# zju3dv/LoG

Measured on NVIDIA H100. Metric: gaussians_per_s_fwd_bwd, higher is better.
Workload: dtype f32

## Files before the change

### include/log_b200_raster.h

```cpp
#ifndef LOG_B200_RASTER_H
#define LOG_B200_RASTER_H

#include <stdint.h>

#ifdef __cplusplus
extern "C" {
#endif

#define LGR_ABI_VERSION 27
#define LGR_TILE 16

#define LGR_FILTER_ADD 0
#define LGR_FILTER_MAX 1
#define LGR_FILTER_NONE 2

#define LGR_E_BADARG (-1)
#define LGR_E_CAPACITY (-2)
#define LGR_E_UNSUPPORTED (-3)

typedef struct lgr_view {
  int32_t image_height, image_width;
  float tanfovx, tanfovy;
  float scale_modifier;
  int32_t sh_degree;
  int32_t sh_coeffs;
  int32_t filter_mode;
  int32_t want_aux;
  int32_t tile_row_begin, tile_row_end;
  int32_t num_owners;
  int32_t raw_params;
  int32_t* band_ids_d;
  int32_t* band_blk_d;
  int32_t* band_count_d;
  int32_t* band_rows_d;
  float* band_dsplat_d;
  int32_t* tile_rank_d;
  const int64_t* gather_index_d;
  const int32_t* pid_map_d;
  int32_t* contrib_id_d;
  uint32_t* contrib_entry_d;
  int32_t* contrib_count_d;
  const int32_t* last_contrib_d;
  const int32_t* region_count_d;
  int64_t region_cap;
  int32_t num_regions;
  int32_t num_channels;
  int32_t log_depth;
  float* splat_ext_d;
  const float* cov3D_precomp_d;
  float* dcov3D_d;
  const float* viewmatrix_d;
  const float* projmatrix_d;
  const float* campos_d;
  const float* bg_d;
} lgr_view;

#define LGR_SPLAT_FLOATS 12
#define LGR_GRAD_FLOATS 12
#define LGR_TILE_SCRATCH_INTS 33
#define LGR_CONTRIB_MAX_LIST (1 << 24)
#define LGR_META_INTS 8

int lgr_abi_version(void);

int lgr_compute_radius(int64_t n, const float* means3D_d, const float* scales_d, const float* rotations_d,
                       const float* projmatrix_d, const float* viewmatrix_d, float focal_x, float focal_y,
                       float tan_fovx, float tan_fovy, float* radii_d, void* stream);

int lgr_mark_visible(int64_t n, const float* means3D_d, const float* viewmatrix_d, uint8_t* visible_d, void* stream);

int lgr_forward_project(const lgr_view* view, int64_t n, const float* means3D_d, const float* opacities_d,
                        const float* scales_d, const float* rotations_d, const float* colors_precomp_d,
                        const float* shs_d, float* splat_d, int32_t* radii_d, uint8_t* clamped_d,
                        int32_t* tile_start_d, int32_t* tile_cursor_d, int32_t* meta_d, void* stream);

int lgr_forward_render(const lgr_view* view, int64_t n, int64_t num_instances, int32_t max_tile_len,
                       int32_t num_long_tiles, const float* splat_d, const int32_t* radii_d, const int32_t* tile_start_d,
                       int32_t* tile_cursor_d, uint32_t* inst_key_d, uint32_t* inst_val_d, uint32_t* inst_tmp_d,
                       int32_t* sorted_ids_d, float* image_d, float* final_T_d, int32_t* n_contrib_d,
                       int32_t* point_id_pixel_d, float* point_weight_pixel_d, float* point_weight_d,
                       int32_t* point_count_d, void* stream);
int32_t lgr_sort_smem_capacity(void);

int lgr_forward_render_device_sized(const lgr_view* view, int64_t n, int64_t instance_capacity, int32_t* meta_d,
                                    const float* splat_d, const int32_t* radii_d, int32_t* tile_start_d,
                                    int32_t* tile_cursor_d, uint32_t* inst_key_d, uint32_t* inst_val_d,
                                    uint32_t* inst_tmp_d, int32_t* sorted_ids_d, float* image_d, float* final_T_d, int32_t* n_contrib_d,
// ... 231 lines not shown
```

### log_b200/_capi.py

```python
import ctypes
import os

from .build import LIB_PATH

_i32, _i64, _f32, _vp = ctypes.c_int32, ctypes.c_int64, ctypes.c_float, ctypes.c_void_p

LGR_FILTER_ADD, LGR_FILTER_MAX, LGR_FILTER_NONE = 0, 1, 2
LGR_SPLAT_FLOATS = 12
LGR_GRAD_FLOATS = 12
LGR_META_INTS = 8
LGR_TILE_SCRATCH_INTS = 33
LGR_ABI_VERSION = 27
LGR_CONTRIB_MAX_LIST = 1 << 24
LGR_STAGE_HEADER_FLOATS = 64
LGR_ROW_FLOATS = 20

EXPORTS = ('lgr_abi_version', 'lgr_sort_smem_capacity', 'lgr_compute_radius', 'lgr_forward_project',
           'lgr_forward_render', 'lgr_forward_render_device_sized', 'lgr_backward', 'lgr_grad_scatter_add', 'lgr_grad_scatter_add_staged', 'lgr_point_compact', 'lgr_sparse_adam', 'lgr_profile_enable', 'lgr_profile_collect',
           'lgr_profile_kernel_name', 'lgr_shard_send', 'lgr_shard_recv_bin', 'lgr_blend_backward', 'lgr_shard_return_rows',
           'lgr_shard_gather', 'lgr_shard_recv_bin_aux', 'lgr_shard_return_packed', 'lgr_shard_gather_packed', 'lgr_tree_traverse', 'lgr_mark_visible',
           'lgr_ssim_forward', 'lgr_ssim_backward', 'lgr_depth_loss_forward', 'lgr_depth_loss_backward', 'lgr_depth_vis',
           'lgr_counter_update', 'lgr_log_step', 'lgr_prepare_cull', 'lgr_prepare_select', 'lgr_photometric_forward',
           'lgr_photometric_backward', 'lgr_corrector_step', 'lgr_densify_plan', 'lgr_densify_map', 'lgr_densify_children',
           'lgr_densify_gather', 'lgr_step_order')
LGR_SHARD_MAX_RANKS = 32
LGR_PROFILE_KERNELS = 12


class LgrView(ctypes.Structure):
    _fields_ = [('image_height', _i32), ('image_width', _i32), ('tanfovx', _f32), ('tanfovy', _f32),
                ('scale_modifier', _f32), ('sh_degree', _i32), ('sh_coeffs', _i32), ('filter_mode', _i32),
                ('want_aux', _i32), ('tile_row_begin', _i32), ('tile_row_end', _i32),
                ('num_owners', _i32), ('raw_params', _i32), ('band_ids_d', _vp), ('band_blk_d', _vp), ('band_count_d', _vp), ('band_rows_d', _vp), ('band_dsplat_d', _vp), ('tile_rank_d', _vp), ('gather_index_d', _vp), ('pid_map_d', _vp), ('contrib_id_d', _vp), ('contrib_entry_d', _vp), ('contrib_count_d', _vp), ('last_contrib_d', _vp),
                ('region_count_d', _vp), ('region_cap', _i64), ('num_regions', _i32), ('num_channels', _i32), ('log_depth', _i32), ('splat_ext_d', _vp), ('cov3D_precomp_d', _vp), ('dcov3D_d', _vp),
                ('viewmatrix_d', _vp), ('projmatrix_d', _vp), ('campos_d', _vp), ('bg_d', _vp)]


class LgrShardLayout(ctypes.Structure):
    _fields_ = [('num_ranks', _i32), ('my_rank', _i32), ('cap', _i64), ('off_count', _i64), ('off_splat', _i64),
                ('off_radii', _i64), ('off_gid', _i64), ('off_dsplat', _i64), ('off_weight', _i64), ('off_pcount', _i64)]


class LgrTree(ctypes.Structure):
    _fields_ = [('num_points', _i64), ('num_nodes', _i64), ('max_child', _i32), ('max_level', _i32),
                ('node_index_d', _vp), ('tree_d', _vp)]


def tree_scratch_ints(num_points, slots):
    return 8 + 2 * num_points + slots + 2 * ((slots + 255) // 256) + 2 + (slots + 3) // 4


class LgrPrepare(ctypes.Structure):
    _fields_ = [('num_points', _i64), ('num_roots', _i64), ('xyz_d', _vp), ('full_proj_d', _vp), ('bound_lo', _f32),
                ('bound_hi', _f32), ('root_index_d', _vp), ('node_index_d', _vp), ('depth_d', _vp), ('opt_all_levels', _i32),
                ('current_depth', _i32), ('flag_d', _vp), ('in_range_d', _vp), ('roots_d', _vp), ('index_all_d', _vp),
                ('leaf_d', _vp), ('node_d', _vp), ('result_d', _vp), ('scratch_d', _vp)]


LGR_PREPARE_RESULTS = 8
(LGR_PREPARE_IN_RANGE, LGR_PREPARE_ROOTS, LGR_PREPARE_WALK, LGR_PREPARE_LEAVES, LGR_PREPARE_NODES, LGR_PREPARE_STATUS,
 LGR_PREPARE_INSTANCES, LGR_PREPARE_OVERFLOW) = range(8)
LGR_PREPARE_ROOT_ORDER = 1


def prepare_scratch_ints(num_points, slots):
    return 2 * num_points + 2 * ((num_points + 255) // 256) + 2 + (num_points + 3) // 4 + tree_scratch_ints(num_points, slots)


# ... 206 lines not shown
```

### log_b200/csrc/lgr_capi.cu

```cuda
#include "lgr_common.cuh"
#include "lgr_prof.cuh"
#include <math.h>

namespace lgr {
int launch_mark_visible(int64_t, const float*, const float*, uint8_t*, cudaStream_t);
int launch_compute_radius(int64_t, const float*, const float*, const float*, const float*, const float*, float, float,
                          float, float, float*, cudaStream_t);
int launch_project_fwd(const View&, Colour, bool, int64_t, const float*, const float*, const float*, const float*,
                       const float*, const float*, float*, int32_t*, uint8_t*, int32_t*, int32_t*, cudaStream_t);
int launch_project_bwd(const View&, Colour, bool, bool, int64_t, const float*, const float*, const float*, const float*,
                       const float*, const int32_t*, const uint8_t*, const float*, float*, float*, float*, float*, float*,
                       float*, float*, float*, void* const*, int, cudaStream_t);
int launch_grad_scatter_add(int64_t, const float*, int64_t, int64_t, float*, cudaStream_t);
int launch_grad_scatter_add_staged(const float*, int, int64_t, int64_t, int64_t, float*, cudaStream_t);
int launch_band_scan(const View&, cudaStream_t);
int launch_tile_scan(int, int32_t*, int32_t*, int32_t*, bool, cudaStream_t);
int launch_bin_and_sort(const View&, int64_t, int64_t, int, int, const float*, const int32_t*, int32_t*, int32_t*,
                        uint32_t*, uint32_t*, uint32_t*, int32_t*, int32_t*, cudaStream_t);
int sort_smem_capacity();
int launch_blend_fwd(const View&, const int32_t*, const int32_t*, const float*, float*, float*, int32_t*, int32_t*,
                     float*, float*, int32_t*, cudaStream_t);
int launch_sparse_adam(int64_t, int, const int64_t*, const float*, float*, float*, float*, float*, float, float, float, float,
                       float, float, float, cudaStream_t);
int launch_counter_update(const lgr_counter&, int64_t, int64_t, const int64_t*, const int64_t*, const int32_t*, const float*,
                          const float*, const int64_t*, int64_t, const void*, const void*, int, int, uint8_t*, cudaStream_t);
int launch_log_step(const lgr_step&, int64_t, int64_t, const int64_t*, const int64_t*, const uint8_t*, cudaStream_t);
int launch_step_order(int64_t, int64_t, int64_t, const int64_t*, const int64_t*, const uint8_t*, int32_t*, int64_t*, cudaStream_t);
int launch_point_compact(int64_t, const int32_t*, int32_t*, int32_t*, int32_t*, int32_t*, cudaStream_t);
int launch_blend_bwd(const View&, const int32_t*, const int32_t*, const float*, const float*, const float*, float*,
                     cudaStream_t);
int launch_shard_send(const View&, const ShardLayout&, int64_t, int64_t, const float*, const int32_t*, int32_t*, void* const*,
                      cudaStream_t);
int launch_shard_recv_count(const View&, const ShardLayout&, float*, float*, int32_t*, int32_t*, float*, int32_t*, cudaStream_t);
int launch_shard_return_packed(const ShardLayout&, const float*, const float*, const float*, const int32_t*, void* const*, cudaStream_t);
int launch_shard_return(const ShardLayout&, const float*, int64_t, const void*, int, int64_t, void* const*, cudaStream_t);
int launch_shard_gather(const View&, const ShardLayout&, int64_t, const float*, const int32_t*, const int32_t*, const float*,
                        float*, float*, int32_t*, int, cudaStream_t);
int launch_tree_traverse(const TreeArgs&, int64_t, int64_t, const int64_t*, int64_t, const int64_t*, int, int32_t*, int64_t*, int64_t*,
                         cudaStream_t);
int launch_prepare_cull(const lgr_prepare&, cudaStream_t);
int launch_prepare_select(const lgr_prepare&, const TreeArgs&, int64_t, int, const float*, const int32_t*, cudaStream_t);
int launch_ssim_fwd(int, int, int, int, const float*, const int64_t*, const float*, const int64_t*, double*, float*, float*,
// ... 190 lines not shown
}

int lgr_backward(const lgr_view* view, int64_t n, int64_t num_instances, const float* means3D_d,
                 const float* opacities_d, const float* scales_d, const float* rotations_d,
                 const float* colors_precomp_d, const float* shs_d, const float* splat_d, const int32_t* radii_d,
                 const uint8_t* clamped_d, const int32_t* tile_start_d, const int32_t* sorted_ids_d,
                 const float* image_d, const float* dL_dimage_d, float* dsplat_d,
                 float* dmeans3D_d, float* dmeans2D_d, float* dopacities_d, float* dscales_d, float* drotations_d,
                 float* dcolors_d, float* dshs_d, float* grad_rows_d, void* const* peer_stage_d, int32_t my_rank,
                 int64_t num_rows, void* stream) {
  if (!view_ok(view) || n < 0 || !tile_start_d || !image_d || !dL_dimage_d) return LGR_E_BADARG;
  if (const int rc6 = six_channels_check(view)) return rc6;
  const bool rows_mode = grad_rows_d || peer_stage_d;
  if (view->num_channels == 6 && rows_mode) return LGR_E_UNSUPPORTED;
  Colour c;
  if (const int rc = colour_source(view, n, colors_precomp_d, shs_d, &c)) return rc;
  if (n == 0) return 0;
  if (c == Colour::LOG_SH && (!dshs_d || !view->campos_d || view->num_owners > 0)) return LGR_E_BADARG;
  const bool cov3d = view->cov3D_precomp_d != nullptr;
  if (!means3D_d || (!cov3d && (!scales_d || !rotations_d)) || !splat_d || !radii_d || !dsplat_d) return LGR_E_BADARG;
  if (cov3d && (!view->dcov3D_d || view->raw_params || view->num_owners > 0 || grad_rows_d || peer_stage_d)) return LGR_E_BADARG;
  if (view->raw_params && (!opacities_d || c == Colour::SH)) return LGR_E_BADARG;
  if (rows_mode) {
    if (view->num_owners <= 0 || c == Colour::SH) return LGR_E_BADARG;
    if (peer_stage_d && (my_rank < 0 || my_rank >= view->num_owners)) return LGR_E_BADARG;
    if (num_rows < 0 || num_rows > n) return LGR_E_BADARG;
  } else {
    if (view->num_owners > 0) return LGR_E_BADARG;
    if (!dmeans3D_d || !dmeans2D_d || !dopacities_d || (!cov3d && (!dscales_d || !drotations_d))) return LGR_E_BADARG;
    if (c == Colour::SH ? (!dshs_d || !clamped_d || !view->campos_d) : !dcolors_d) return LGR_E_BADARG;
  }
  if (num_instances > 0 && !sorted_ids_d) return LGR_E_BADARG;
  cudaStream_t st = (cudaStream_t)stream;
  const View v = make_view(view, n);
  int rc = 0;
  if (num_instances > 0) rc = launch_blend_bwd(v, tile_start_d, sorted_ids_d, splat_d, image_d, dL_dimage_d, dsplat_d, st);
  if (rc) return rc;
  return launch_project_bwd(v, c, cov3d, rows_mode, rows_mode ? num_rows : n, means3D_d, opacities_d, scales_d, rotations_d, shs_d, radii_d, clamped_d, dsplat_d,
                            dmeans3D_d, dmeans2D_d, dopacities_d, dscales_d, drotations_d, dcolors_d, dshs_d, grad_rows_d, peer_stage_d, my_rank, st);
}

int lgr_sparse_adam(int64_t rows, int32_t row_floats, const int64_t* index_d, const float* grad_d, float* param_d,
                    float* exp_avg_d, float* exp_avg_sq_d, float* max_exp_avg_sq_d, int64_t step, double lr, double beta1,
                    double beta2, double eps, void* stream) {
  if (rows < 0 || row_floats <= 0 || step < 1) return LGR_E_BADARG;
  if (rows > 0 && (!index_d || !grad_d || !param_d || !exp_avg_d || !exp_avg_sq_d)) return LGR_E_BADARG;
  Residence where;
  where.on_device(param_d); where.on_device(index_d); where.on_device(grad_d);
  where.state(exp_avg_d); where.state(exp_avg_sq_d); where.state(max_exp_avg_sq_d);
  if (!where.ok) return LGR_E_BADARG;
  const double bc1 = 1.0 - pow(beta1, (double)step), bc2 = 1.0 - pow(beta2, (double)step);
  const double step_size = lr / bc1;
  return launch_sparse_adam(rows, row_floats, index_d, grad_d, param_d, exp_avg_d, exp_avg_sq_d, max_exp_avg_sq_d,
                            (float)beta1, (float)beta2, (float)(1.0 - beta1), (float)(1.0 - beta2), (float)sqrt(bc2),
                            (float)(-step_size), (float)eps, (cudaStream_t)stream);
}

int lgr_counter_update(const lgr_counter* counter, int64_t num_leaf, int64_t num_node, const int64_t* index_leaf_d,
                       const int64_t* index_node_d, const int32_t* radii_d, const float* point_weight_d, const float* grad_d,
                       const int64_t* grad_strides, int64_t num_points, const void* point_id_d, const void* point_count_d,
                       int32_t id_bytes, int32_t count_bytes, uint8_t* flag_vis_d, void* stream) {
  if (!counter || num_leaf < 0 || num_node < 0 || num_points < 0 || !grad_strides) return LGR_E_BADARG;
  if ((id_bytes != 4 && id_bytes != 8) || (count_bytes != 4 && count_bytes != 8)) return LGR_E_BADARG;
  if ((num_leaf > 0 && !index_leaf_d) || (num_node > 0 && !index_node_d)) return LGR_E_BADARG;
  const lgr_counter& c = *counter;
  if (!c.create_steps_d || !c.visible_count_d || !c.weights_max_d || !c.weights_sum_d || !c.radii_max_d || !c.area_sum_d ||
      !c.grad_sum_d || !c.radii_max_max_d)
    return LGR_E_BADARG;
// ... 416 lines not shown
```

### log_b200/csrc/lgr_common.cuh

```cuda
#pragma once
#include <cuda_runtime.h>
#include <stdint.h>

#include "../../include/log_b200_raster.h"

namespace lgr {

constexpr int TILE = LGR_TILE;
constexpr int TILE_PIX = TILE * TILE;
constexpr float NEAR_Z = 0.2f;
constexpr float ALPHA_MAX = 0.99f;
constexpr float ALPHA_MIN = 1.0f / 255.0f;
constexpr float T_STOP = 1e-4f;
constexpr float FILTER_VAR = 0.3f;
constexpr float CLAMP_FOV = 1.3f;
constexpr int CSTRIDE = 32;
constexpr float LOG2E = 1.4426950408889634f;
constexpr float LN2 = 0.6931471805599453f;
constexpr int COMPACT_CHUNK = 256;

enum class Colour { RGB, SH, LOG_SH, RGB6 };

struct View {
  int H, W, gx, gy;
  int row0, row1;
  float tanfovx, tanfovy, fx, fy, scale_mod;
  int sh_degree, sh_K, filter_mode, want_aux;
  int raw_params;
  int num_owners, owner_chunk;
  int32_t* band_ids;
  int32_t* band_blk;
  int32_t* band_count;
  int32_t* band_rows;
  float* band_dsplat;
  const int64_t* gather;
  const int32_t* pid_map;
  int32_t* contrib_id;
  uint32_t* contrib_entry;
  int32_t* contrib_count;
  const int32_t* last_contrib;
  const int32_t* region_count;
  int64_t region_cap;
  int regions;
  const float* cov3d;
  float* dcov3d;
  int band_blocks;
  const float* view;
  const float* proj;
  const float* campos;
  const float* bg;
  int num_channels;
  int log_depth;
  float* splat_ext;
};

inline View make_view(const lgr_view* v, int64_t n = 0) {
  View o;
  o.num_owners = v->num_owners; o.band_ids = v->band_ids_d; o.band_blk = v->band_blk_d; o.band_count = v->band_count_d; o.band_rows = v->band_rows_d; o.band_dsplat = v->band_dsplat_d; o.gather = v->gather_index_d; o.pid_map = v->pid_map_d; o.contrib_id = v->contrib_id_d; o.contrib_entry = v->contrib_entry_d; o.contrib_count = v->contrib_count_d; o.last_contrib = v->last_contrib_d;
  o.region_count = v->region_count_d; o.region_cap = v->region_cap; o.regions = v->region_count_d ? v->num_regions : 0;
  o.cov3d = v->cov3D_precomp_d; o.dcov3d = v->dcov3D_d;
  o.owner_chunk = o.num_owners > 0 ? (int)LGR_OWNER_CHUNK(n, (int64_t)o.num_owners) : 256;
  if (o.owner_chunk < 256) o.owner_chunk = 256;
  o.band_blocks = (int)((n + 255) / 256);
  o.H = v->image_height; o.W = v->image_width;
  o.gx = (o.W + TILE - 1) / TILE; o.gy = (o.H + TILE - 1) / TILE;
  o.row0 = v->tile_row_begin; o.row1 = v->tile_row_end;
  if (o.row0 == 0 && o.row1 == 0) o.row1 = o.gy;
  o.tanfovx = v->tanfovx; o.tanfovy = v->tanfovy;
  o.fx = o.W / (2.0f * v->tanfovx); o.fy = o.H / (2.0f * v->tanfovy);
  o.scale_mod = v->scale_modifier;
  o.sh_degree = v->sh_degree; o.sh_K = v->sh_coeffs; o.filter_mode = v->filter_mode; o.want_aux = v->want_aux;
  o.raw_params = v->raw_params;
  o.view = v->viewmatrix_d; o.proj = v->projmatrix_d; o.campos = v->campos_d; o.bg = v->bg_d;
  o.num_channels = v->num_channels == 6 ? 6 : 3; o.splat_ext = v->splat_ext_d; o.log_depth = v->log_depth ? 1 : 0;
  return o;
}

struct ShardLayout {
  int R, me;
  int64_t cap;
  int64_t off_count, off_splat, off_radii, off_gid, off_dsplat, off_weight, off_pcount;
};

struct TreeArgs {
  const int32_t* node_index;
  const int32_t* tree;
  int C;
  const float* xyz;
  const float* scaling_raw;
  const float* rotation_raw;
  const float* view;
  const float* proj;
  float fx, fy, tanfovx, tanfovy, min_px;
};


__device__ __forceinline__ float4 ldg4(const float* p) { return __ldg(reinterpret_cast<const float4*>(p)); }

struct Cov2D {
  float a, b, c;
  float a_raw, c_raw;
  float t[3];
  float T[6];
  bool inx, iny;
};

__device__ __forceinline__ void quat_to_R(const float4 q, float R[9]) {
// ... 179 lines not shown
```

### log_b200/csrc/lgr_project.cu

```cuda
#include "lgr_common.cuh"
#include "lgr_prof.cuh"

namespace lgr {

constexpr int PROJ_THREADS = 256;

__device__ __forceinline__ void load3(const float* __restrict__ p, int64_t i, float o[3]) {
  o[0] = __ldg(p + 3 * i); o[1] = __ldg(p + 3 * i + 1); o[2] = __ldg(p + 3 * i + 2);
}

__device__ __forceinline__ void load_cov3d(const float* cov, int64_t i, float Sg[9]) {
  const float* c6 = cov + 6 * i;
  const float cxx = __ldg(c6), cxy = __ldg(c6 + 1), cxz = __ldg(c6 + 2), cyy = __ldg(c6 + 3), cyz = __ldg(c6 + 4), czz = __ldg(c6 + 5);
  Sg[0] = cxx; Sg[1] = cxy; Sg[2] = cxz; Sg[3] = cxy; Sg[4] = cyy; Sg[5] = cyz; Sg[6] = cxz; Sg[7] = cyz; Sg[8] = czz;
}

__device__ __forceinline__ void sh_dir_basis(const float p[3], const float* cam, int deg, float B[16]) {
  const float d[3] = {p[0] - cam[0], p[1] - cam[1], p[2] - cam[2]};
  const float inv = 1.0f / sqrtf(d[0] * d[0] + d[1] * d[1] + d[2] * d[2]);
  sh_basis(deg, d[0] * inv, d[1] * inv, d[2] * inv, B);
}

__device__ __forceinline__ void sh_accumulate(const float* sh, const float B[16], int first, int nb, float rgb[3]) {
  for (int k = first; k < nb; k++) {
// ... 239 lines not shown
template <Colour C, bool COV3D, bool DEPTH, bool ROWS>
__global__ void __launch_bounds__(PROJ_THREADS)
project_bwd_kernel(View v, int64_t n, const float* __restrict__ means, const float* __restrict__ opac,
                   const float* __restrict__ scales, const float* __restrict__ rots, const float* __restrict__ shs, const int32_t* __restrict__ radii,
                   const uint8_t* __restrict__ clamped, const float* __restrict__ dsplat, float* __restrict__ dmeans,
                   float* __restrict__ dmeans2D, float* __restrict__ dopac, float* __restrict__ dscales,
                   float* __restrict__ drots, float* __restrict__ dcolors, float* __restrict__ dshs,
                   float* __restrict__ grad_rows, void* const* __restrict__ peer_stage, int my_rank) {
  static_assert(!(C == Colour::RGB6 && DEPTH), "the depth pass generates channels 3..5: colours are (N,3)");
  static_assert(!(C == Colour::LOG_SH && COV3D), "LoG's raw parameters come with scales and rotations");
  static_assert(!ROWS || (C == Colour::RGB && !COV3D && !DEPTH), "band mode rows carry three precomputed colours only");
  constexpr bool USE_SH = C == Colour::SH, LOG_SH = C == Colour::LOG_SH, SIX = C == Colour::RGB6;
  __shared__ float sV[16], sP[16], sCam[3];
  if (threadIdx.x < 16) { sV[threadIdx.x] = v.view[threadIdx.x]; sP[threadIdx.x] = v.proj[threadIdx.x]; }
  if ((USE_SH || LOG_SH) && threadIdx.x < 3) sCam[threadIdx.x] = v.campos[threadIdx.x];
  __syncthreads();
  int64_t blk = blockIdx.x;
  if (ROWS && peer_stage) {
    int64_t first = 0;
    for (int o = 0; o <= my_rank && o < v.num_owners - 1; o++) first += v.band_count[o];
    if (my_rank == v.num_owners - 1) first = 0;
    blk = (blk + first / PROJ_THREADS) % gridDim.x;
  }
  int64_t i = blk * PROJ_THREADS + threadIdx.x;
  const bool active = i < n;
  if (!ROWS && !active) return;
  int64_t row = 0;
  if (ROWS && active) {
    row = i;
    i = v.band_rows[row];
  }
  float dm[3] = {0.f, 0.f, 0.f}, dm2[2] = {0.f, 0.f}, dop = 0.f, dsc[3] = {0.f, 0.f, 0.f}, dq[4] = {0.f, 0.f, 0.f, 0.f};
  float drgb[3] = {0.f, 0.f, 0.f}, dext[3] = {0.f, 0.f, 0.f};
  const bool live = active && radii[i] > 0;
  const int64_t src = (v.gather && live) ? v.gather[i] : i;
  const int K = v.sh_K;
  if (live) {
    const float4 g0 = ldg4(dsplat + i * LGR_GRAD_FLOATS);
    const float4 g1 = ldg4(dsplat + i * LGR_GRAD_FLOATS + 4);
    const float4 g2 = ldg4(dsplat + i * LGR_GRAD_FLOATS + 8);
    float p[3], s0[3], s[3], R[9], Sg[9];
    load3(means, src, p);
    float4 q = make_float4(1.f, 0.f, 0.f, 0.f);
    float q_inv = 1.0f;
    if (COV3D) {
      load_cov3d(v.cov3d, src, Sg);
    } else {
      load3(scales, src, s0);
      q = ldg4(rots + 4 * src);
      if (v.raw_params) {
#pragma unroll
        for (int k = 0; k < 3; k++) s0[k] = expf(s0[k]);
        q = act_normalize(q, q_inv);
      }
#pragma unroll
      for (int k = 0; k < 3; k++) s[k] = s0[k] * v.scale_mod;
      quat_to_R(q, R);
      cov3d(s, R, Sg);
    }
    Cov2D cv;
    cov2d(sV, p, Sg, v.fx, v.fy, v.tanfovx, v.tanfovy, v.filter_mode, cv);
    dop = g1.y;
    drgb[0] = g1.z; drgb[1] = g1.w; drgb[2] = g2.x;
    if (SIX) { dext[0] = g2.y; dext[1] = g2.z; dext[2] = g2.w; }
    const float a = cv.a, b = cv.b, c = cv.c;
    const float det = a * c - b * b, idet2 = 1.0f / (det * det);
    float da = idet2 * (-c * c * g0.z + b * c * g0.w + (det - a * c) * g1.x);
// ... 167 lines not shown
      }
      float4* sr = s_rows + threadIdx.x * 5;
      sr[0] = make_float4(dm[0], dm[1], dm[2], dm2[0]);
      sr[1] = make_float4(dm2[1], 0.f, dop, dsc[0]);
      sr[2] = make_float4(dsc[1], dsc[2], dq[0], dq[1]);
      sr[3] = make_float4(dq[2], dq[3], drgb[0], drgb[1]);
      sr[4] = make_float4(drgb[2], __int_as_float((int)i), (float)radii[i], 0.f);
      s_dst[threadIdx.x] = dst;
    }
    __syncthreads();
    const int64_t left = n - blk * PROJ_THREADS;
    const int cnt = left < PROJ_THREADS ? (int)left : PROJ_THREADS;
    for (int idx = threadIdx.x; idx < cnt * 5; idx += PROJ_THREADS) {
      const int r = idx / 5;
      s_dst[r][idx - 5 * r] = s_rows[idx];
    }
    return;
  }
  dmeans[3 * i] = dm[0]; dmeans[3 * i + 1] = dm[1]; dmeans[3 * i + 2] = dm[2];
  dmeans2D[3 * i] = dm2[0]; dmeans2D[3 * i + 1] = dm2[1]; dmeans2D[3 * i + 2] = 0.f;
  dopac[i] = dop;
  if (!COV3D) {
    dscales[3 * i] = dsc[0]; dscales[3 * i + 1] = dsc[1]; dscales[3 * i + 2] = dsc[2];
    reinterpret_cast<float4*>(drots)[i] = make_float4(dq[0], dq[1], dq[2], dq[3]);
  }
  if (SIX) {
    float* dc = dcolors + 6 * i;
    dc[0] = drgb[0]; dc[1] = drgb[1]; dc[2] = drgb[2]; dc[3] = dext[0]; dc[4] = dext[1]; dc[5] = dext[2];
  } else if (!USE_SH) {
    dcolors[3 * i] = drgb[0]; dcolors[3 * i + 1] = drgb[1]; dcolors[3 * i + 2] = drgb[2];
  }
}

__global__ void __launch_bounds__(1024)
band_scan_kernel(View v) {
  __shared__ int warp_sum[32];
  __shared__ int carry_s;
  const int tid = threadIdx.x, lane = tid & 31, wid = tid >> 5, B = v.band_blocks;
  if (tid == 0) carry_s = 0;
  __syncthreads();
  for (int base = 0; base < B; base += 1024) {
    const int b = base + tid;
    const int c = b < B ? v.band_blk[b] : 0;
    int x = c;
#pragma unroll
    for (int o = 1; o < 32; o <<= 1) { const int y = __shfl_up_sync(0xffffffffu, x, o); if (lane >= o) x += y; }
    if (lane == 31) warp_sum[wid] = x;
    __syncthreads();
    if (wid == 0) {
      int w = warp_sum[lane];
#pragma unroll
      for (int o = 1; o < 32; o <<= 1) { const int y = __shfl_up_sync(0xffffffffu, w, o); if (lane >= o) w += y; }
      warp_sum[lane] = w;
    }
    __syncthreads();
    const int carry = carry_s;
    if (b < B) v.band_blk[B + b] = carry + (wid ? warp_sum[wid - 1] : 0) + x - c;
    __syncthreads();
    if (tid == 1023) carry_s = carry + warp_sum[31];
    __syncthreads();
  }
  if (tid == 0) v.band_blk[2 * B] = carry_s;
  __syncthreads();
  const int cpb = v.owner_chunk / PROJ_THREADS;
  for (int o = tid; o < v.num_owners; o += 1024) {
    const int b0 = min(B, o * cpb), b1 = min(B, (o + 1) * cpb);
// ... 140 lines not shown
```

### log_b200/rasterizer.py

```python
import ctypes
from typing import NamedTuple, Optional

import torch
import torch.nn as nn

from . import _capi
from ._capi import LGR_FILTER_ADD, LGR_FILTER_MAX, LGR_FILTER_NONE, LgrView

CONTRIB_BITS = bool(int(__import__('os').environ.get('LGR_CONTRIB_BITS', '1')))
FLAVOUR_STOCK = 'stock'
FLAVOUR_FORK = 'fork'


class GaussianRasterizationSettings(NamedTuple):
    image_height: int
    image_width: int
    tanfovx: float
    tanfovy: float
    bg: torch.Tensor
    scale_modifier: float
    viewmatrix: torch.Tensor
    projmatrix: torch.Tensor
    sh_degree: int
    campos: torch.Tensor
# ... 127 lines not shown
                'lgr_forward_project')
    return splat, radii, clamped, tile_start, tile_cursor, meta


def render(view, n, splat, radii, tile_start, tile_cursor, meta, image, final_T, n_contrib, pid, pwp, pw, pc, alloc,
           capacity=None, stats=None):
    lib = _capi.load()
    ntiles = _view_tiles(view)
    if capacity:
        D, max_len = int(capacity), None
    else:
        D, max_len = stats['num_instances'], stats['max_tile_len']
        if D < 0 or stats['stock_instances'] > 0x7fffffff:
            raise _capi.LgrError(f'this view needs {stats["stock_instances"]} (Gaussian, tile) instances by the stock rule '
                                 f'(D = {D & 0xffffffff} binned, {stats["num_visible"]} of {n} Gaussians visible, longest tile '
                                 f'list {max_len}): more than 2^31 - 1 is unsupported')
    inst_key = alloc('inst_key', (D,), torch.int32)
    inst_val = alloc('inst_val', (D,), torch.int32)
    inst_tmp = alloc('inst_tmp', (2 * D,), torch.int32)
    sorted_ids = alloc('sorted_ids', (D,), torch.int32)
    contrib = alloc('contrib', (2 * D + ntiles,), torch.int32) if use_contrib_lists(D, max_len) else None
    set_contrib_lists(view, contrib, D, n_contrib)
    buffers = (_ptr(splat), _ptr(radii), _ptr(tile_start), _ptr(tile_cursor), _ptr(inst_key), _ptr(inst_val), _ptr(inst_tmp),
               _ptr(sorted_ids), _ptr(image), _ptr(final_T), _ptr(n_contrib), _ptr(pid), _ptr(pwp), _ptr(pw), _ptr(pc),
               _stream(image.device))
    if capacity:
        _capi.check(lib.lgr_forward_render_device_sized(ctypes.byref(view), n, D, _ptr(meta), *buffers),
                    'lgr_forward_render_device_sized')
    else:
        _capi.check(lib.lgr_forward_render(ctypes.byref(view), n, D, max_len, stats['num_long_tiles'], *buffers), 'lgr_forward_render')
    return sorted_ids, contrib


def backward_per_gaussian(view, n, num_instances, params, splat, radii, clamped, tile_start, sorted_ids, image, grad_image, dsplat):
    means3D, opacities, scales, rotations, colors_precomp, shs = params
    f32 = dict(dtype=torch.float32, device=means3D.device)
    cov = scales is None
    dmeans3D, dmeans2D, dopac = torch.empty((n, 3), **f32), torch.empty((n, 3), **f32), torch.empty((n,), **f32)
    dscales = None if cov else torch.empty((n, 3), **f32)
    drot = None if cov else torch.empty((n, 4), **f32)
    dcov3D = torch.empty((n, 6), **f32) if cov else None
    if cov:
        view.dcov3D_d = dcov3D.data_ptr()
    dcolors = torch.empty((n, int(colors_precomp.shape[-1])), **f32) if colors_precomp is not None else None
    dshs = torch.empty((n,) + tuple(shs.shape[1:]), **f32) if shs is not None else None
    _capi.check(_capi.load().lgr_backward(ctypes.byref(view), n, num_instances, _ptr(means3D), _ptr(opacities), _ptr(scales),
                                          _ptr(rotations), _ptr(colors_precomp), _ptr(shs), _ptr(splat), _ptr(radii),
                                          _ptr(clamped), _ptr(tile_start), _ptr(sorted_ids), _ptr(image), _ptr(grad_image),
                                          _ptr(dsplat), _ptr(dmeans3D), _ptr(dmeans2D), _ptr(dopac), _ptr(dscales), _ptr(drot),
                                          _ptr(dcolors), _ptr(dshs), None, None, 0, 0, _stream(means3D.device)), 'lgr_backward')
    return (dmeans3D, dmeans2D, dopac, dscales, drot, dcolors, dshs), dcov3D


class RasterState:
    __slots__ = ('view', 'keep', 'n', 'num_instances', 'max_tile_len', 'stock_instances', 'num_visible', 'splat',
                 'radii', 'clamped', 'tile_start', 'sorted_ids', 'final_T', 'n_contrib', 'image', 'sh', 'num_owners',
                 'dsplat', 'band_counts_host', 'point_count', 'meta', 'cov3D', 'dcov3D', 'contrib', 'splat_ext')

    def read_stats(self):
        return decode_meta(self.meta.tolist())

    def contrib_lists(self):
        if self.contrib is None:
            return None
        D = self.num_instances
        return self.contrib[:D], self.contrib[D:2 * D], self.contrib[2 * D:]


def rasterize_forward(settings, means3D, opacities, scales, rotations, colors_precomp, shs, filter_mode, want_aux,
                      tile_rows=None, num_owners=0, raw_params=False, gather_index=None, instance_capacity=None,
                      cov3D_precomp=None, log_depth=False):
    channels = colour_channels(colors_precomp, settings, shs, raw_params, gather_index, num_owners, log_depth)
    if log_depth:
        bg3 = settings.bg.reshape(-1)[:3]
        settings = settings._replace(bg=torch.cat([bg3, bg3]))
    dev = means3D.device
    if cov3D_precomp is not None and (raw_params or num_owners > 0):
        raise _capi.LgrError('cov3D_precomp is not available with raw_params or in band mode')
    for name, t in (('opacities', opacities), ('scales', scales), ('rotations', rotations), ('colors_precomp', colors_precomp),
                    ('shs', shs), ('cov3D_precomp', cov3D_precomp), ('viewmatrix', settings.viewmatrix), ('projmatrix', settings.projmatrix), ('bg', settings.bg)):
        if t is not None and t.device != dev:
            raise _capi.LgrError(f'{name} is on {t.device}, means3D on {dev}: all inputs of a call must share one device')
    n = int(means3D.shape[0])
    keep = []
    if gather_index is not None:
        if gather_index.dtype != torch.int64 or gather_index.device != dev or gather_index.dim() != 1:
            raise _capi.LgrError('gather_index must be a 1-D int64 tensor on the inputs\' device')
        if num_owners > 0:
            raise _capi.LgrError('gather_index is not available in band mode')
        gather_index = gather_index.contiguous()
# ... 19 lines not shown
    splat, radii, clamped, tile_start, tile_cursor, meta = project(view, n, alloc, means3D, opacities, scales, rotations,
                                                                   colors_precomp, shs)
    H, W = view.image_height, view.image_width
    image = torch.empty((channels, H, W), **f32) if tile_rows is None else torch.zeros((channels, H, W), **f32)
    final_T = torch.empty((H, W), **f32) if tile_rows is None else torch.ones((H, W), **f32)
    n_contrib = torch.empty((H, W), **i32) if tile_rows is None else torch.zeros((H, W), **i32)
    pid = pwp = pw = pc = None
    if want_aux:
        pc = torch.zeros((n,), **i32)
        pid = torch.empty((H, W), **i32) if tile_rows is None else torch.full((H, W), -1, **i32)
        pwp = torch.empty((H, W), **f32) if tile_rows is None else torch.zeros((H, W), **f32)
        pw = torch.zeros((n,), **f32)
    m = stats = None
    if instance_capacity:
        if num_owners > 0:
            raise _capi.LgrError('instance_capacity (device-sized call) is not available in band mode')
    else:
        m = (meta if band_count is None else torch.cat([meta, band_count])).tolist()
        stats = decode_meta(m)
    sorted_ids, contrib = render(view, n, splat, radii, tile_start, tile_cursor, meta, image, final_T, n_contrib, pid, pwp, pw, pc,
                                 alloc, instance_capacity, stats)
    keep.append(contrib)
    s = RasterState()
    s.view, s.keep, s.n, s.meta = view, keep, n, meta
    if stats is None:
        s.num_instances, s.max_tile_len, s.stock_instances, s.num_visible = int(instance_capacity), None, None, None
    else:
        s.num_instances, s.max_tile_len = stats['num_instances'], stats['max_tile_len']
        s.stock_instances, s.num_visible = stats['stock_instances'], stats['num_visible']
    s.cov3D, s.dcov3D = cov3D_precomp, None
    s.splat, s.radii, s.clamped, s.tile_start, s.sorted_ids = splat, radii, clamped, tile_start, sorted_ids
    s.final_T, s.n_contrib, s.image, s.sh = final_T, n_contrib, image, shs is not None
    s.point_count = pc
    s.contrib = contrib
    s.splat_ext = splat_ext
    s.num_owners, s.dsplat = num_owners, band_dsplat
    s.band_counts_host = [int(x) for x in m[_capi.LGR_META_INTS:]] if num_owners > 0 else None
    return image, radii, pid, pwp, pw, s


def rasterize_backward(state: RasterState, grad_image, means3D, opacities, scales, rotations, colors_precomp, shs,
                       peer_stage=None, my_rank=0):
    dev = means3D.device
    n = state.n
    g = _f32c(grad_image, 'grad_image', dev)
    dsplat, state.dsplat = state.dsplat, None
    if dsplat is None:
        dsplat = torch.zeros((n, _capi.LGR_GRAD_FLOATS), dtype=torch.float32, device=dev)
    if state.num_owners == 0:
        grads, state.dcov3D = backward_per_gaussian(state.view, n, state.num_instances, (means3D, opacities, scales, rotations,
                                                    colors_precomp, shs), state.splat, state.radii, state.clamped,
                                                    state.tile_start, state.sorted_ids, state.image, g, dsplat)
        return grads
    m_rows = sum(state.band_counts_host)
    rows = None if peer_stage is not None else torch.empty((m_rows, _capi.LGR_ROW_FLOATS), dtype=torch.float32, device=dev)
    grad_rows = None if rows is None else _ptr(rows) if rows.numel() else _ptr(dsplat)
    _capi.check(_capi.load().lgr_backward(ctypes.byref(state.view), n, state.num_instances, _ptr(means3D), _ptr(opacities),
                                          _ptr(scales), _ptr(rotations), _ptr(colors_precomp), None, _ptr(state.splat),
                                          _ptr(state.radii), None, _ptr(state.tile_start), _ptr(state.sorted_ids),
                                          _ptr(state.image), _ptr(g), _ptr(dsplat), None, None, None, None, None, None, None,
                                          grad_rows, _ptr(peer_stage), int(my_rank) if peer_stage is not None else 0, m_rows,
                                          _stream(dev)), 'lgr_backward')
    return rows


def point_id_count(point_count: torch.Tensor):
    lib = _capi.load()
    n = int(point_count.shape[0])
    dev = point_count.device
    i32 = dict(dtype=torch.int32, device=dev)
    scratch = torch.empty((2 * ((n + 1023) // 1024) + 1,), **i32)
    ids = torch.empty((n,), **i32)
    cnt = torch.empty((n,), **i32)
    num = torch.empty((1,), **i32)
    _capi.check(lib.lgr_point_compact(n, _ptr(point_count), _ptr(scratch), _ptr(ids), _ptr(cnt),
                                      ctypes.c_void_p(num.data_ptr()), _stream(dev)), 'lgr_point_compact')
    k = int(num.item())
    return ids[:k], cnt[:k]


class _RasterizeGaussians(torch.autograd.Function):

    @staticmethod
    def forward(ctx, means3D, means2D, opacities, colors_precomp, shs, scales, rotations, settings, filter_mode, want_aux,
                tile_rows, raw_params=False, instance_capacity=None, holder=None, cov3D_precomp=None, log_depth=False):
# ... 112 lines not shown
```

### profiles/contrib_stats.py

```python
import argparse
import json
import os
import sys

import numpy as np
import torch

ROOT = os.path.dirname(os.path.dirname(os.path.abspath(__file__)))
sys.path.insert(0, ROOT)

BATCH = 256


def main():
    ap = argparse.ArgumentParser()
    ap.add_argument('--workload', default='10m')
    args = ap.parse_args()
    from bench import WORKLOADS, make_inputs
    from log_b200 import GaussianRasterizationSettings, rasterize_forward
    from log_b200._capi import LGR_FILTER_MAX
    n, W, H, _, deg = WORKLOADS[args.workload]
    dev = torch.device('cuda')
    cam, sc, _ = make_inputs(args.workload)
    d = {k: v.to(dev) for k, v in sc.items()}
    settings = GaussianRasterizationSettings(
        image_height=H, image_width=W, tanfovx=cam.tanfovx, tanfovy=cam.tanfovy, bg=cam.bg.to(dev), scale_modifier=1.0,
        viewmatrix=cam.viewmatrix.to(dev), projmatrix=cam.projmatrix.to(dev), sh_degree=deg, campos=cam.campos.to(dev),
        prefiltered=False, debug=False)
    *_, st = rasterize_forward(settings, d['means3D'], d['opacities'].reshape(-1), d['scales'], d['rotations'],
                               d['colors'] if deg == 0 else None, d['shs'] if deg > 0 else None, LGR_FILTER_MAX, True)
    torch.cuda.synchronize()
    count = st.contrib_lists()[2].cpu().numpy().astype(np.int64)
    start = st.tile_start.cpu().numpy().astype(np.int64)
    nc = st.n_contrib.cpu().numpy()
    gx, gy = (W + 15) // 16, (H + 15) // 16
    pad = np.zeros((gy * 16, gx * 16), np.int64)
    pad[:H, :W] = nc
    maxlast = pad.reshape(gy, 16, gx, 16).max(axis=(1, 3)).reshape(-1)
    lens = start[1:] - start[:-1]
    used = lens > 0
    b_before = np.where(used, np.maximum(1, (maxlast + BATCH - 1) // BATCH), 0)
    staged = np.minimum(lens, b_before * BATCH)
    nz_staged = count[:len(lens)]
    assert (nz_staged <= staged).all()
    b_after = (nz_staged + BATCH - 1) // BATCH
    entry = st.contrib_lists()[1].cpu().numpy().view(np.uint32)
    ntiles = len(lens)
    cnt = nz_staged
    pos = np.repeat(start[:ntiles], cnt) + (np.arange(cnt.sum()) - np.repeat(np.cumsum(cnt) - cnt, cnt))
    byte = (entry[pos] & 0xff).astype(np.uint8)
    bits = np.unpackbits(byte[:, None], axis=1, bitorder='little')
    tile_of = np.repeat(np.arange(ntiles), cnt)
    hits_tw = np.zeros((ntiles, 8), np.int64)
    np.add.at(hits_tw, tile_of, bits.astype(np.int64))
    busy = hits_tw.sum(axis=1) > 0
    imb = hits_tw[busy].max(axis=1) / hits_tw[busy].mean(axis=1)
    hits = int(hits_tw.sum())
    out = {
        'workload': args.workload, 'gpu': torch.cuda.get_device_name(), 'instances': int(lens.sum()),
        'tiles': int(len(lens)), 'tiles_with_entries': int(used.sum()),
        'staged_entries': int(staged.sum()), 'nonzero_staged_entries': int(nz_staged.sum()),
        'zero_share_of_staged': float(1.0 - nz_staged.sum() / max(staged.sum(), 1)),
        'staged_share_of_list': float(staged.sum() / max(lens.sum(), 1)),
        'batches_per_tile_before': {'mean': float(b_before[used].mean()), 'max': int(b_before.max()), 'total': int(b_before.sum())},
        'batches_per_tile_after': {'mean': float(b_after[used].mean()), 'max': int(b_after.max()), 'total': int(b_after.sum())},
        'warp_hits': hits, 'warp_hits_per_entry': float(hits / max(int(cnt.sum()), 1)),
        'vector_reds': {'per_warp_hit': 3 * hits, 'per_entry': 3 * int(cnt.sum())},
        'slowest_warp_over_mean': {'mean': float(imb.mean()), 'p50': float(np.median(imb)), 'p90': float(np.percentile(imb, 90)),
                                   'hit_weighted': float((hits_tw[busy].max(axis=1) * 8).sum() / max(hits, 1))},
        'entries_per_warp_tile': {'mean': float(cnt[busy].mean()), 'max': int(cnt.max()),
                                  'hits_per_warp_tile_mean': float(hits_tw[busy].mean())},
    }
    print(json.dumps(out))


if __name__ == '__main__':
    main()
```

Measured before the change: 1.929 billion.

## Skip backward projection and dsplat zeroing for uncomposited gaussians using point weights

Passes the forward pass's per-point compositing weight into the backward pass. Visible gaussians whose weight is zero are treated as not live in projection backward, so their parameter rows are never read. The full dsplat zero-fill is replaced by a kernel that zeroes only the 32-byte sectors touching rows with nonzero weight. This cuts memory traffic for visible gaussians that contribute nothing, at the cost of an extra weight read, a version check on the Python side, and a more complex correctness contract for unzeroed gradient rows.

```diff
diff --git a/include/log_b200_raster.h b/include/log_b200_raster.h
--- a/include/log_b200_raster.h
+++ b/include/log_b200_raster.h
@@ -7,7 +7,7 @@
 extern "C" {
 #endif
 
-#define LGR_ABI_VERSION 27
+#define LGR_ABI_VERSION 28
 #define LGR_TILE 16
 
 #define LGR_FILTER_ADD 0
@@ -53,6 +53,8 @@
   const float* projmatrix_d;
   const float* campos_d;
   const float* bg_d;
+  const float* live_weight_d;
+  int32_t dsplat_unzeroed;
 } lgr_view;
 
 #define LGR_SPLAT_FLOATS 12
diff --git a/log_b200/_capi.py b/log_b200/_capi.py
--- a/log_b200/_capi.py
+++ b/log_b200/_capi.py
@@ -10,7 +10,7 @@
 LGR_GRAD_FLOATS = 12
 LGR_META_INTS = 8
 LGR_TILE_SCRATCH_INTS = 33
-LGR_ABI_VERSION = 27
+LGR_ABI_VERSION = 28
 LGR_CONTRIB_MAX_LIST = 1 << 24
 LGR_STAGE_HEADER_FLOATS = 64
 LGR_ROW_FLOATS = 20
@@ -33,7 +33,8 @@
                 ('want_aux', _i32), ('tile_row_begin', _i32), ('tile_row_end', _i32),
                 ('num_owners', _i32), ('raw_params', _i32), ('band_ids_d', _vp), ('band_blk_d', _vp), ('band_count_d', _vp), ('band_rows_d', _vp), ('band_dsplat_d', _vp), ('tile_rank_d', _vp), ('gather_index_d', _vp), ('pid_map_d', _vp), ('contrib_id_d', _vp), ('contrib_entry_d', _vp), ('contrib_count_d', _vp), ('last_contrib_d', _vp),
                 ('region_count_d', _vp), ('region_cap', _i64), ('num_regions', _i32), ('num_channels', _i32), ('log_depth', _i32), ('splat_ext_d', _vp), ('cov3D_precomp_d', _vp), ('dcov3D_d', _vp),
-                ('viewmatrix_d', _vp), ('projmatrix_d', _vp), ('campos_d', _vp), ('bg_d', _vp)]
+                ('viewmatrix_d', _vp), ('projmatrix_d', _vp), ('campos_d', _vp), ('bg_d', _vp), ('live_weight_d', _vp),
+                ('dsplat_unzeroed', _i32)]
 
 
 class LgrShardLayout(ctypes.Structure):
diff --git a/log_b200/csrc/lgr_capi.cu b/log_b200/csrc/lgr_capi.cu
--- a/log_b200/csrc/lgr_capi.cu
+++ b/log_b200/csrc/lgr_capi.cu
@@ -8,6 +8,7 @@
                           float, float, float*, cudaStream_t);
 int launch_project_fwd(const View&, Colour, bool, int64_t, const float*, const float*, const float*, const float*,
                        const float*, const float*, float*, int32_t*, uint8_t*, int32_t*, int32_t*, cudaStream_t);
+int launch_zero_live_rows(const View&, int64_t, float*, cudaStream_t);
 int launch_project_bwd(const View&, Colour, bool, bool, int64_t, const float*, const float*, const float*, const float*,
                        const float*, const int32_t*, const uint8_t*, const float*, float*, float*, float*, float*, float*,
                        float*, float*, float*, void* const*, int, cudaStream_t);
@@ -264,8 +265,17 @@
   }
   if (num_instances > 0 && !sorted_ids_d) return LGR_E_BADARG;
   cudaStream_t st = (cudaStream_t)stream;
-  const View v = make_view(view, n);
+  View v = make_view(view, n);
+  if (view->live_weight_d && num_instances > 0 && !rows_mode && view->want_aux) {
+    v.live_weight = view->live_weight_d;
+    v.list_total = tile_start_d + v.gx * (v.row1 - v.row0);
+  }
   int rc = 0;
+  if (view->dsplat_unzeroed) {
+    rc = v.live_weight ? launch_zero_live_rows(v, n, dsplat_d, st)
+                       : (int)cudaMemsetAsync(dsplat_d, 0, sizeof(float) * LGR_GRAD_FLOATS * (size_t)n, st);
+    if (rc) return rc;
+  }
   if (num_instances > 0) rc = launch_blend_bwd(v, tile_start_d, sorted_ids_d, splat_d, image_d, dL_dimage_d, dsplat_d, st);
   if (rc) return rc;
   return launch_project_bwd(v, c, cov3d, rows_mode, rows_mode ? num_rows : n, means3D_d, opacities_d, scales_d, rotations_d, shs_d, radii_d, clamped_d, dsplat_d,
diff --git a/log_b200/csrc/lgr_common.cuh b/log_b200/csrc/lgr_common.cuh
--- a/log_b200/csrc/lgr_common.cuh
+++ b/log_b200/csrc/lgr_common.cuh
@@ -52,6 +52,8 @@
   int num_channels;
   int log_depth;
   float* splat_ext;
+  const float* live_weight;
+  const int32_t* list_total;
 };
 
 inline View make_view(const lgr_view* v, int64_t n = 0) {
@@ -73,6 +75,7 @@
   o.raw_params = v->raw_params;
   o.view = v->viewmatrix_d; o.proj = v->projmatrix_d; o.campos = v->campos_d; o.bg = v->bg_d;
   o.num_channels = v->num_channels == 6 ? 6 : 3; o.splat_ext = v->splat_ext_d; o.log_depth = v->log_depth ? 1 : 0;
+  o.live_weight = nullptr; o.list_total = nullptr;
   return o;
 }
 
diff --git a/log_b200/csrc/lgr_project.cu b/log_b200/csrc/lgr_project.cu
--- a/log_b200/csrc/lgr_project.cu
+++ b/log_b200/csrc/lgr_project.cu
@@ -295,7 +295,8 @@
   }
   float dm[3] = {0.f, 0.f, 0.f}, dm2[2] = {0.f, 0.f}, dop = 0.f, dsc[3] = {0.f, 0.f, 0.f}, dq[4] = {0.f, 0.f, 0.f, 0.f};
   float drgb[3] = {0.f, 0.f, 0.f}, dext[3] = {0.f, 0.f, 0.f};
-  const bool live = active && radii[i] > 0;
+  bool live = active && radii[i] > 0;
+  if (!ROWS && live && v.live_weight && __ldg(v.live_weight + i) == 0.f && __ldg(v.list_total) > 0) live = false;
   const int64_t src = (v.gather && live) ? v.gather[i] : i;
   const int K = v.sh_K;
   if (live) {
@@ -529,6 +530,32 @@
   }
 }
 
+__global__ void __launch_bounds__(PROJ_THREADS)
+zero_live_rows_kernel(int64_t sectors, const float* __restrict__ weight, const int32_t* __restrict__ list_total,
+                      float4* __restrict__ dsplat) {
+  const int64_t s = (int64_t)blockIdx.x * PROJ_THREADS + threadIdx.x;
+  if (s >= sectors) return;
+  constexpr int ROW = 4 * LGR_GRAD_FLOATS;
+  const int64_t r0 = 32 * s / ROW, r1 = (32 * s + 31) / ROW;
+  if (__ldg(list_total) > 0 && __ldg(weight + r0) == 0.f && __ldg(weight + r1) == 0.f) return;
+  dsplat[2 * s] = dsplat[2 * s + 1] = make_float4(0.f, 0.f, 0.f, 0.f);
+}
+
+int launch_zero_live_rows(const View& v, int64_t n, float* dsplat, cudaStream_t st) {
+  if (n == 0) return 0;
+  const int64_t sectors = n * LGR_GRAD_FLOATS * 4 / 32;
+  const unsigned blocks = (unsigned)((sectors + PROJ_THREADS - 1) / PROJ_THREADS);
+  if (sectors > 0) {
+    zero_live_rows_kernel<<<blocks, PROJ_THREADS, 0, st>>>(sectors, v.live_weight, v.list_total, reinterpret_cast<float4*>(dsplat));
+    LGR_CHECK_LAUNCH();
+  }
+  if (n & 1) {
+    cudaError_t e = cudaMemsetAsync(dsplat + (n * LGR_GRAD_FLOATS - 4), 0, 16, st);
+    if (e != cudaSuccess) return (int)e;
+  }
+  return 0;
+}
+
 __global__ void __launch_bounds__(1024)
 band_scan_kernel(View v) {
   __shared__ int warp_sum[32];
diff --git a/log_b200/rasterizer.py b/log_b200/rasterizer.py
--- a/log_b200/rasterizer.py
+++ b/log_b200/rasterizer.py
@@ -183,7 +183,8 @@
     return sorted_ids, contrib
 
 
-def backward_per_gaussian(view, n, num_instances, params, splat, radii, clamped, tile_start, sorted_ids, image, grad_image, dsplat):
+def backward_per_gaussian(view, n, num_instances, params, splat, radii, clamped, tile_start, sorted_ids, image, grad_image, dsplat,
+                          live_weight=None, unzeroed=False):
     means3D, opacities, scales, rotations, colors_precomp, shs = params
     f32 = dict(dtype=torch.float32, device=means3D.device)
     cov = scales is None
@@ -195,18 +196,30 @@
         view.dcov3D_d = dcov3D.data_ptr()
     dcolors = torch.empty((n, int(colors_precomp.shape[-1])), **f32) if colors_precomp is not None else None
     dshs = torch.empty((n,) + tuple(shs.shape[1:]), **f32) if shs is not None else None
-    _capi.check(_capi.load().lgr_backward(ctypes.byref(view), n, num_instances, _ptr(means3D), _ptr(opacities), _ptr(scales),
-                                          _ptr(rotations), _ptr(colors_precomp), _ptr(shs), _ptr(splat), _ptr(radii),
-                                          _ptr(clamped), _ptr(tile_start), _ptr(sorted_ids), _ptr(image), _ptr(grad_image),
-                                          _ptr(dsplat), _ptr(dmeans3D), _ptr(dmeans2D), _ptr(dopac), _ptr(dscales), _ptr(drot),
-                                          _ptr(dcolors), _ptr(dshs), None, None, 0, 0, _stream(means3D.device)), 'lgr_backward')
+    view.live_weight_d = _ptr(live_weight)
+    view.dsplat_unzeroed = int(unzeroed)
+    try:
+        _capi.check(_capi.load().lgr_backward(ctypes.byref(view), n, num_instances, _ptr(means3D), _ptr(opacities), _ptr(scales),
+                                              _ptr(rotations), _ptr(colors_precomp), _ptr(shs), _ptr(splat), _ptr(radii),
+                                              _ptr(clamped), _ptr(tile_start), _ptr(sorted_ids), _ptr(image), _ptr(grad_image),
+                                              _ptr(dsplat), _ptr(dmeans3D), _ptr(dmeans2D), _ptr(dopac), _ptr(dscales), _ptr(drot),
+                                              _ptr(dcolors), _ptr(dshs), None, None, 0, 0, _stream(means3D.device)), 'lgr_backward')
+    finally:
+        view.live_weight_d, view.dsplat_unzeroed = None, 0
     return (dmeans3D, dmeans2D, dopac, dscales, drot, dcolors, dshs), dcov3D
 
 
 class RasterState:
     __slots__ = ('view', 'keep', 'n', 'num_instances', 'max_tile_len', 'stock_instances', 'num_visible', 'splat',
                  'radii', 'clamped', 'tile_start', 'sorted_ids', 'final_T', 'n_contrib', 'image', 'sh', 'num_owners',
-                 'dsplat', 'band_counts_host', 'point_count', 'meta', 'cov3D', 'dcov3D', 'contrib', 'splat_ext')
+                 'dsplat', 'band_counts_host', 'point_count', 'meta', 'cov3D', 'dcov3D', 'contrib', 'splat_ext', 'point_weight',
+                 'point_weight_version')
+
+    def live_weight(self):
+        pw = self.point_weight
+        if pw is None or self.num_owners > 0 or pw._version != self.point_weight_version:
+            return None
+        return pw
 
     def read_stats(self):
         return decode_meta(self.meta.tolist())
@@ -292,6 +305,7 @@
     s.splat, s.radii, s.clamped, s.tile_start, s.sorted_ids = splat, radii, clamped, tile_start, sorted_ids
     s.final_T, s.n_contrib, s.image, s.sh = final_T, n_contrib, image, shs is not None
     s.point_count = pc
+    s.point_weight, s.point_weight_version = pw, (pw._version if pw is not None else None)
     s.contrib = contrib
     s.splat_ext = splat_ext
     s.num_owners, s.dsplat = num_owners, band_dsplat
@@ -305,12 +319,17 @@
     n = state.n
     g = _f32c(grad_image, 'grad_image', dev)
     dsplat, state.dsplat = state.dsplat, None
-    if dsplat is None:
+    live_weight = state.live_weight() if state.num_owners == 0 else None
+    unzeroed = dsplat is None and live_weight is not None
+    if unzeroed:
+        dsplat = torch.empty((n, _capi.LGR_GRAD_FLOATS), dtype=torch.float32, device=dev)
+    elif dsplat is None:
         dsplat = torch.zeros((n, _capi.LGR_GRAD_FLOATS), dtype=torch.float32, device=dev)
     if state.num_owners == 0:
         grads, state.dcov3D = backward_per_gaussian(state.view, n, state.num_instances, (means3D, opacities, scales, rotations,
                                                     colors_precomp, shs), state.splat, state.radii, state.clamped,
-                                                    state.tile_start, state.sorted_ids, state.image, g, dsplat)
+                                                    state.tile_start, state.sorted_ids, state.image, g, dsplat,
+                                                    live_weight=live_weight, unzeroed=unzeroed)
         return grads
     m_rows = sum(state.band_counts_host)
     rows = None if peer_stage is not None else torch.empty((m_rows, _capi.LGR_ROW_FLOATS), dtype=torch.float32, device=dev)
diff --git a/profiles/contrib_stats.py b/profiles/contrib_stats.py
--- a/profiles/contrib_stats.py
+++ b/profiles/contrib_stats.py
@@ -15,19 +15,22 @@
 def main():
     ap = argparse.ArgumentParser()
     ap.add_argument('--workload', default='10m')
+    ap.add_argument('--order', default='random', choices=['random', 'morton'])
     args = ap.parse_args()
-    from bench import WORKLOADS, make_inputs
+    from bench import WORKLOADS, make_inputs, morton_order
     from log_b200 import GaussianRasterizationSettings, rasterize_forward
     from log_b200._capi import LGR_FILTER_MAX
     n, W, H, _, deg = WORKLOADS[args.workload]
     dev = torch.device('cuda')
     cam, sc, _ = make_inputs(args.workload)
+    if args.order == 'morton':
+        sc = morton_order(cam, sc, W, H)
     d = {k: v.to(dev) for k, v in sc.items()}
     settings = GaussianRasterizationSettings(
         image_height=H, image_width=W, tanfovx=cam.tanfovx, tanfovy=cam.tanfovy, bg=cam.bg.to(dev), scale_modifier=1.0,
         viewmatrix=cam.viewmatrix.to(dev), projmatrix=cam.projmatrix.to(dev), sh_degree=deg, campos=cam.campos.to(dev),
         prefiltered=False, debug=False)
-    *_, st = rasterize_forward(settings, d['means3D'], d['opacities'].reshape(-1), d['scales'], d['rotations'],
+    _, radii, _, _, pw, st = rasterize_forward(settings, d['means3D'], d['opacities'].reshape(-1), d['scales'], d['rotations'],
                                d['colors'] if deg == 0 else None, d['shs'] if deg > 0 else None, LGR_FILTER_MAX, True)
     torch.cuda.synchronize()
     count = st.contrib_lists()[2].cpu().numpy().astype(np.int64)
@@ -71,7 +74,34 @@
         'entries_per_warp_tile': {'mean': float(cnt[busy].mean()), 'max': int(cnt.max()),
                                   'hits_per_warp_tile_mean': float(hits_tw[busy].mean())},
     }
+    out['order'] = args.order
+    out['skip'] = skip_model(radii, pw, deg)
     print(json.dumps(out))
+
+
+def skip_model(radii, pw, deg):
+    vis = radii > 0
+    live = vis & (pw > 0)
+    n = int(radii.numel())
+    rows = {'dsplat': 48, 'means3D': 12, 'scales': 12, 'rotations': 16}
+    if deg > 0:
+        rows['shs'] = 4 * 3 * (deg + 1) ** 2
+    model = {}
+    for name, b in rows.items():
+        def sectors(mask):
+            idx = torch.nonzero(mask).reshape(-1).to(torch.int64)
+            first, last = idx * b // 32, (idx * b + b - 1) // 32
+            hit = torch.zeros(((n * b + 31) // 32,), dtype=torch.bool, device=radii.device)
+            for k in range(int((b + 31) // 32) + 1):
+                s = torch.minimum(first + k, last)
+                hit[s] = True
+            return int(hit.sum())
+        before, after = sectors(vis), sectors(live)
+        model[name] = {'row_bytes': b, 'sectors_before': before, 'sectors_after': after,
+                       'unread_share': 1.0 - after / max(before, 1), 'bytes_saved': 32 * (before - after)}
+    nv, nl = int(vis.sum()), int(live.sum())
+    return {'visible': nv, 'composited': nl, 'not_composited': nv - nl, 'f': (nv - nl) / max(nv, 1),
+            'bytes_saved_total': sum(m['bytes_saved'] for m in model.values()), 'arrays': model}
 
 
 if __name__ == '__main__':
```

Result: faster. 1.952 billion, median of 6 (+1.2%).
